# GiulioRomualdi/paper_romualdi_2022_icra_centroidal-mpc-walking

Hardware: AMD Instinct MI355X
Metric: centroidal-MPC solves/sec (batch, horizon=20) (higher is better)
Workload: dtype f32

## Files before the change

### include/cmpc.h

```cpp
#ifndef CMPC_H
#define CMPC_H

#include <stddef.h>

#ifdef __cplusplus
extern "C" {
#endif

typedef struct cmpc_handle_s* cmpc_handle;

typedef enum {
    CMPC_OK = 0,
    CMPC_ERR_ARG = -1,
    CMPC_ERR_HIP = -2,
    CMPC_ERR_NOT_CONVERGED = -3
} cmpc_status;

typedef struct {
    int horizon;
    double sampling_time;
    double friction_coefficient;
    double gravity;
    double com_weight[3];
    double angular_momentum_weight;
// ... 22 lines not shown
void cmpc_default_config(cmpc_config* cfg);
int cmpc_dims(int horizon, int* n_x, int* n_p, int* n_g, int* nnz_jac, int* nnz_hess);

double cmpc_default_tolerance(int horizon);
int cmpc_create(const cmpc_config* cfg, int batch, int device, cmpc_handle* out);
int cmpc_destroy(cmpc_handle h);
const char* cmpc_last_error(cmpc_handle h);
int cmpc_batch(cmpc_handle h);
void* cmpc_stream(cmpc_handle h);

int cmpc_solve_device(cmpc_handle h, const float* dP, const float* dX0, float* dX, float* dInfo,
                      void* stream);
int cmpc_solve_device_warm(cmpc_handle h, const float* dP, const float* dX0, float* dX, float* dInfo,
                           void* stream);
int cmpc_set_warm_policy(cmpc_handle h, int warm_budget, int restart_in_kernel);
int cmpc_solve(cmpc_handle h, const float* P, const float* X0, float* X, float* info);
float cmpc_last_solve_ms(cmpc_handle h);
int cmpc_set_timing(cmpc_handle h, int enabled);
int cmpc_test_poison_lds(cmpc_handle h);

typedef struct {
    double friction_coefficient;
    double com_weight[3];
    double angular_momentum_weight;
    double contact_position_weight;
    double force_rate_of_change_weight[3];
    double contact_force_symmetry_weight;
    double corners[2][4][3];
} cmpc_model;
#define CMPC_MODEL_DOUBLES 34
// ... 137 lines not shown
```

### paper_romualdi_2022_icra_centroidal-mpc-walking_amd/_capi.py

```python
from __future__ import annotations

import ctypes as C
import os

_HERE = os.path.dirname(os.path.abspath(__file__))
LIB_PATH = os.path.join(_HERE, os.environ.get("CMPC_LIB", "libcmpc_hip.so"))

INFO = 8
CERT = 8
SENS = 8


class CmpcConfig(C.Structure):
    _fields_ = [
        ("horizon", C.c_int),
        ("sampling_time", C.c_double),
        ("friction_coefficient", C.c_double),
        ("gravity", C.c_double),
        ("com_weight", C.c_double * 3),
        ("angular_momentum_weight", C.c_double),
        ("contact_position_weight", C.c_double),
        ("force_rate_of_change_weight", C.c_double * 3),
        ("contact_force_symmetry_weight", C.c_double),
        ("corners", C.c_double * 24),
# ... 49 lines not shown
    "cmpc_batch", "cmpc_stream", "cmpc_solve_device", "cmpc_solve", "cmpc_last_solve_ms", "cmpc_set_timing",
    "cmpc_eval_nlp_device", "cmpc_nlp_sparsity", "cmpc_set_state", "cmpc_set_reference",
    "cmpc_set_contacts", "cmpc_set_initial_guess", "cmpc_advance", "cmpc_get_solution",
    "cmpc_get_output", "cmpc_set_reference_from_planner", "cmpc_plant_step_device", "cmpc_test_poison_lds",
    "cmpc_compact_output_device", "cmpc_contacts_merge", "cmpc_contacts_merge_device", "cmpc_contacts_sample",
    "cmpc_contacts_sample_device", "cmpc_set_contact_lists", "cmpc_contacts_adjust", "cmpc_contacts_adjust_device",
    "cmpc_write_state_device", "cmpc_shift_solution_device", "cmpc_eval_nlp_grad_device", "cmpc_solve_device_warm", "cmpc_set_warm_policy",
    "cmpc_get_parameters", "cmpc_get_parameters_device", "cmpc_allgather_compact_device",
    "cmpc_rollout_tick_device", "cmpc_write_reference_from_planner_device", "cmpc_default_tolerance",
    "cmpc_contacts_force_sample_time", "cmpc_contacts_force_sample_time_device",
    "cmpc_model_from_config", "cmpc_check_models", "cmpc_set_models", "cmpc_set_models_device",
    "cmpc_set_multiplier_output", "cmpc_get_multipliers_device", "cmpc_get_multipliers", "cmpc_kkt_certificate_device",
    "cmpc_value_gradient_device", "cmpc_solution_jvp_device", "cmpc_solution_vjp_device",
    "cmpc_sensitivity_workspace_bytes", "cmpc_solution_jvp_model_device", "cmpc_solution_vjp_model_device", "cmpc_model_value_gradient_device",
    "cmpc_plant_step_jvp_device", "cmpc_plant_step_vjp_device", "cmpc_contacts_position_vjp_device", "cmpc_rollout_tick_vjp_device",
]

_lib = None


def lib():
    global _lib
    if _lib is None:
        if not os.path.exists(LIB_PATH):
            raise RuntimeError(
                f"{LIB_PATH} not found: build it with `python -c 'import __graft_entry__ as g; g.build()'` "
                "(hipcc --offload-arch=gfx950). This package has no CPU fallback.")
        try:
            import torch
        except ImportError:
# ... 62 lines not shown
            L.cmpc_solution_jvp_model_device.argtypes = [vp, fp, fp, fp, fp, vp, C.c_int, fp, fp, vp]
            L.cmpc_solution_vjp_model_device.argtypes = [vp, fp, fp, fp, fp, fp, vp, fp, vp]
            L.cmpc_model_value_gradient_device.argtypes = [vp, fp, fp, fp, vp, vp]
        L.cmpc_plant_step_jvp_device.argtypes = [vp, fp, fp, fp, d, i, vp, fp, fp, vp, vp, vp]
        L.cmpc_plant_step_vjp_device.argtypes = [vp, fp, fp, fp, d, i, vp, vp, fp, fp, vp, vp]
        L.cmpc_contacts_position_vjp_device.argtypes = [vp, i, d, i, i] + [vp] * 15
        L.cmpc_rollout_tick_vjp_device.argtypes = [vp, i, d, C.POINTER(CmpcTickTape)] + [vp] * 11
        if hasattr(L, "cmpc_get_parameters"):
            L.cmpc_get_parameters.argtypes = [vp, fp]
            L.cmpc_get_parameters_device.argtypes = [vp, C.POINTER(vp)]
            L.cmpc_allgather_compact_device.argtypes = [vp, vp, C.c_int, fp, fp, vp]
        if hasattr(L, "cmpc_rollout_tick_device"):
            L.cmpc_rollout_tick_device.argtypes = [vp, i, d, i, C.POINTER(CmpcTickIO), vp]
        if hasattr(L, "cmpc_write_reference_from_planner_device"):
            L.cmpc_write_reference_from_planner_device.argtypes = [vp, fp, fp, i, d, d, d, d, fp, vp]
        if hasattr(L, "cmpc_set_models"):
            L.cmpc_model_from_config.argtypes = [C.POINTER(CmpcConfig), C.POINTER(CmpcModel)]
            L.cmpc_model_from_config.restype = None
            L.cmpc_check_models.argtypes = [vp, i]
            L.cmpc_set_models.argtypes = [vp, vp]
            L.cmpc_set_models_device.argtypes = [vp, vp, vp, vp]
        _lib = L
    return _lib
```

### paper_romualdi_2022_icra_centroidal-mpc-walking_amd/csrc/cmpc_api.hip

```cpp
#include "../../include/cmpc.h"
#include "cmpc_contacts.h"
#include "cmpc_device.h"

#include <algorithm>
#include <cmath>
#include <cstdio>
#include <cstdlib>
#include <cstring>
#include <dlfcn.h>
#include <string>
#include <vector>

extern "C" size_t cmpc_solver_lds_bytes(int N, int factors_global);
extern "C" int cmpc_launch_solver(const CmpcParams* prm, size_t lds_bytes, hipStream_t stream);
extern "C" int cmpc_prepare_solver(int N, int factors_global, size_t lds_bytes);
extern "C" int cmpc_launch_nlp_eval(const CmpcParams* prm, const float* dX, const float* dP, const float* dLamG,
                                    float lam_f, float* dF, float* dG, float* dGradF, float* dJac, float* dHess,
                                    hipStream_t stream);
extern "C" int cmpc_launch_nlp_grad(const CmpcParams* prm, const float* dX, const float* dP, const float* dLamG, float lam_f, float* dGradX,
                                    float* dGradP, hipStream_t stream);
extern "C" int cmpc_launch_multipliers(const CmpcParams* prm, const float* dX, const float* dP, float* dLamG, hipStream_t stream);
extern "C" int cmpc_launch_kkt_certificate(const CmpcParams* prm, const float* dX, const float* dP, const float* dLamG, float* dCert, hipStream_t stream);
extern "C" int cmpc_launch_value_gradient(const CmpcParams* prm, const float* dX, const float* dP, const float* dLamG, float* dGradP, hipStream_t stream);
extern "C" int cmpc_launch_sensitivity(const CmpcConsts* kc, int kc_per_problem, int N, int b0, int nb, const float* dX, const float* dP, const float* dLamG,
                                       const float* dDir, const float* dGradX, int kdir, float* dOut, float* dSens, double* dWs, const double* dDirModel,
                                       double* dGradModel, hipStream_t stream);
extern "C" int cmpc_launch_model_value_gradient(const CmpcParams* prm, const float* dX, const float* dP, const float* dLamG, double* dGradModel,
                                                hipStream_t stream);
extern "C" int cmpc_launch_warm_shift(const CmpcParams* prm, const float* dXprev, float* dX0, hipStream_t stream);
extern "C" int cmpc_launch_contacts_merge(int B, int M, double now, const double* plan_t, const float* plan_pose, const int* plan_n,
// ... 37 lines not shown
    CmpcLayout L;
    int B = 0, device = 0;
    hipStream_t stream = nullptr;
    hipEvent_t ev0 = nullptr, ev1 = nullptr;
    bool timed = false;
    bool timing = true;
    float* dP = nullptr;
    float* dX0 = nullptr;
    float* dX = nullptr;
    float* dInfo = nullptr;
    CmpcConsts* dConsts = nullptr;
    double hExpK[CMPC_NMAX + 1];
    double* dExpK = nullptr;
    CmpcConsts* dModels = nullptr;
    bool models_set = false;
    float* dScratch = nullptr;
    float* dBox = nullptr;
    float* dDuals = nullptr;
    bool mult_out = false;
    float* dLamG = nullptr;
    double* dSensWs = nullptr;
    hipEvent_t sens_ev = nullptr;
    double* dSnapT = nullptr;
    int* dSnapOk = nullptr;
    char* dTickWs = nullptr;
    hipEvent_t tick_ev = nullptr;
    size_t snap_cap = 0;
    int warm_duals = 0;
    float hBox[12] = {0};
    bool box_set = false;
// ... 147 lines not shown
    HIPCHK_CREATE(hipMalloc(&h->dConsts, sizeof(CmpcConsts)));
    for (int k = 0; k <= cfg->horizon; ++k) h->hExpK[k] = std::exp(-(double)k);
    HIPCHK_CREATE(hipMalloc(&h->dExpK, sizeof(double) * (cfg->horizon + 1)));
    HIPCHK_CREATE(hipMemcpy(h->dExpK, h->hExpK, sizeof(double) * (cfg->horizon + 1), hipMemcpyHostToDevice));
    HIPCHK_CREATE(hipMalloc(&h->dBox, sizeof(float) * 12));
    if (h->warm_duals) {
        const size_t nd = (size_t)batch * (CMPC_NS * (cfg->horizon + 1) + 2 * CMPC_NI * cfg->horizon);
        HIPCHK_CREATE(hipMalloc(&h->dDuals, sizeof(float) * nd));
        HIPCHK_CREATE(hipMemset(h->dDuals, 0, sizeof(float) * nd));
    }
    {
        CmpcConsts q;
        fill_consts(h, q);
        HIPCHK_CREATE(hipMemcpy(h->dConsts, &q, sizeof(q), hipMemcpyHostToDevice));
    }
    HIPCHK_CREATE(hipDeviceSynchronize());
#undef HIPCHK_CREATE
    *out = h;
    return CMPC_OK;
}

int cmpc_destroy(cmpc_handle h)
{
    if (!h) return CMPC_OK;
    hipSetDevice(h->device);
    if (h->stream) hipStreamSynchronize(h->stream);
    if (h->hXpin) hipHostFree(h->hXpin);
    if (h->hInfoPin) hipHostFree(h->hInfoPin);
    hipFree(h->dP); hipFree(h->dX0); hipFree(h->dX); hipFree(h->dInfo); hipFree(h->dConsts); hipFree(h->dScratch); hipFree(h->dBox); hipFree(h->dDuals); hipFree(h->dLamG); hipFree(h->dSensWs);
    if (h->sens_ev) hipEventDestroy(h->sens_ev);
    hipFree(h->dSnapT); hipFree(h->dSnapOk); hipFree(h->dTickWs); if (h->tick_ev) hipEventDestroy(h->tick_ev); hipFree(h->dExpK); hipFree(h->dModels);
    if (h->ev0) hipEventDestroy(h->ev0);
    if (h->ev1) hipEventDestroy(h->ev1);
    if (h->stream) hipStreamDestroy(h->stream);
    delete h;
    return CMPC_OK;
}

static void fill_consts(cmpc_handle h, CmpcConsts& q)
{
    const cmpc_config& c = h->cfg;
    std::memset(&q, 0, sizeof(q));
    q.N = c.horizon; q.max_iter = c.max_iterations;
    q.exact_hessian = c.exact_hessian; q.final_extrap = c.final_extrapolation;
    q.tail_stages = c.tail_stages; q.tail_iters = c.tail_iterations; q.tail_trigger = (float)c.tail_trigger;
    q.dt = (float)c.sampling_time; q.grav = (float)c.gravity;
// ... 9 lines not shown
    q.sigma_min = 0.03f;
#ifdef CMPC_PROFILE
    if (const char* e = std::getenv("CMPC_SIGMA_MIN")) q.sigma_min = (float)std::atof(e);
    if (const char* e = std::getenv("CMPC_HWID_PROBE")) q.hwid_probe = std::atoi(e);
#endif
}

static const float* model_corners(cmpc_handle h) { return h->models_set ? h->dModels->corners : h->dConsts->corners; }
static int corners_stride(cmpc_handle h) { return h->models_set ? (int)(sizeof(CmpcConsts) / sizeof(float)) : 0; }

static void fill_params(cmpc_handle h, CmpcParams& p)
{
    std::memset(&p, 0, sizeof(p));
    p.kc = h->models_set ? h->dModels : h->dConsts; p.N = h->cfg.horizon; p.B = h->B;
    p.kc_per_problem = h->models_set ? 1 : 0;
    p.scratch = h->dScratch; p.scratch_stride = h->scratch_stride;
    p.mu_init = h->cfg.mu_init > 0 ? (float)h->cfg.mu_init : 0.1f;
    p.mu_adapt = h->cfg.mu_init > 0 ? 0.f : h->mu_adapt;
    p.t_floor = 1e-2f;
    p.warm_budget = h->warm_budget; p.warm_no_restart = h->warm_no_restart;
    p.duals = (h->mult_out || h->warm_duals) ? h->dDuals : nullptr; p.warm_duals = h->warm_duals;
}

static int solve_device_impl(cmpc_handle h, const float* dP, const float* dX0, float* dX, float* dInfo, void* stream, bool warm)
{
    if (!h || !dP || !dX0 || !dX) return fail(h, CMPC_ERR_ARG, "cmpc_solve_device: null argument");
    HIPCHK(h, hipSetDevice(h->device));
    hipStream_t st = stream ? (hipStream_t)stream : h->stream;
    CmpcParams p;
    fill_params(h, p);
    p.P = dP; p.X0 = dX0; p.X = dX; p.info = dInfo ? dInfo : h->dInfo;
    if (warm || h->force_warm) {
        p.mu_init = (float)h->mu_warm; p.mu_adapt = 0.f; p.t_floor = (float)h->floor_warm; p.warm = 1;
    }
    if (h->timing) HIPCHK(h, hipEventRecord(h->ev0, st));
    int rc = cmpc_launch_solver(&p, h->lds, st);
    if (rc != 0) return fail(h, CMPC_ERR_HIP, std::string("solver launch: ") + hipGetErrorString((hipError_t)rc));
    if (h->timing) HIPCHK(h, hipEventRecord(h->ev1, st));
    h->timed = h->timing;
    return CMPC_OK;
}

int cmpc_solve_device(cmpc_handle h, const float* dP, const float* dX0, float* dX, float* dInfo, void* stream)
{
    return solve_device_impl(h, dP, dX0, dX, dInfo, stream, false);
}

int cmpc_set_warm_policy(cmpc_handle h, int warm_budget, int restart_in_kernel)
{
    if (!h || warm_budget < 0) return fail(h, CMPC_ERR_ARG, "cmpc_set_warm_policy: bad argument");
    h->warm_budget = warm_budget;
    h->warm_no_restart = restart_in_kernel ? 0 : 1;
    return CMPC_OK;
}

int cmpc_solve_device_warm(cmpc_handle h, const float* dP, const float* dX0, float* dX, float* dInfo, void* stream)
{
    return solve_device_impl(h, dP, dX0, dX, dInfo, stream, true);
}

// ... 1002 lines not shown
```

### paper_romualdi_2022_icra_centroidal-mpc-walking_amd/csrc/cmpc_device.h

```cpp
#pragma once
#include <hip/hip_runtime.h>

#include "../../include/cmpc.h"

#define CMPC_NS 15
#define CMPC_NF 24
#define CMPC_NQ 6
#define CMPC_NU 30
#define CMPC_NXA 39
#define CMPC_NI 44
#define CMPC_REC_N 1088
#define CMPC_NMAX 40
#define CMPC_TZ_LDS_NMAX 20
#define CMPC_INFO_N 8

struct CmpcLayout {
    int N;
    int p_R[2], p_up[2], p_lo[2], p_gam[2], p_nom[2], p_cur[2];
    int p_com0, p_dcom0, p_h0, p_comref, p_href, p_fext, p_text, np;
    int o_com, o_dcom, o_h, o_pos[2], o_vel[2], o_f[2][4], nx, ng;
};

__host__ __device__ inline void cmpc_layout_init(CmpcLayout& L, int N)
{
// ... 108 lines not shown
    const float* P;
    const float* X0;
    float* X;
    float* info;
    float mu_init, t_floor;
    float mu_adapt;
    int warm;
    int warm_budget;
    int warm_no_restart;
    float* duals;
    int warm_duals;
    float* scratch;
    long long scratch_stride;
    int lds_words;
    int kc_per_problem;
};
```

### paper_romualdi_2022_icra_centroidal-mpc-walking_amd/csrc/cmpc_solver.hip

```cpp
#include "cmpc_device.h"

#include <cstdlib>
#include <type_traits>
#include <map>
#include <mutex>

#define NS CMPC_NS
#define NF CMPC_NF
#define NQ CMPC_NQ
#define NU CMPC_NU
#define NXA CMPC_NXA
#define NI CMPC_NI
#define PLD 39
#define GLD 30
#define RLD 36
#define NPAN 46
#define GEO 36
#define SQ_TILE_WAVES 6
#define SQ_SPIN_MAX (1 << 20)
#define SQ_PUB_FLOATS (10 * NPAN * 4 + 128 * 4)
#define ZLD 36
#define MSET (NU * RLD + NPAN * RLD + NS * 16)
#define NTRI 256
#define ID_STRIP_LEN 68
// ... 63 lines not shown
    float *S, *U, *T, *Z;
    float* LAM;
    float *dS, *dU, *dT, *dZ, *d;
    float *Lf;
    float *geoA;
    float *P0, *Qb, *G, *QuuF, *Pan, *Bval, *Aval, *arow, *ybuf, *fpv, *fpn;
    float *idstrip;
    float *ZT;
    double *QuuD1, *qs1;
    int *Brow, *Arow, *qmask;
    unsigned short* tri;
    double *QuuD, *pv, *pn, *qs, *Pd, *sig, *gco, *redd;
    float* red;
    int* flag;
    int* prog;
};

__device__ inline void wave_lds_sync() { asm volatile("" ::: "memory"); }
typedef __attribute__((address_space(3))) const float* ldsf_t;
typedef __attribute__((address_space(3))) float* ldsw_t;
__device__ inline ldsf_t lds_opaque(const float* p) { ldsf_t q = (ldsf_t)p; asm volatile("" : "+v"(q)); return q; }
__device__ inline ldsw_t lds_opaque_w(float* p) { ldsw_t q = (ldsw_t)p; asm volatile("" : "+v"(q)); return q; }
typedef float v4f __attribute__((ext_vector_type(4)));
typedef float v2f __attribute__((ext_vector_type(2)));
__device__ inline float4 lds_ld4(ldsf_t p)
{
    const v4f v = *reinterpret_cast<__attribute__((address_space(3))) const v4f*>(p);
    return make_float4(v[0], v[1], v[2], v[3]);
}

// ... 73 lines not shown
    if (!FG) { c.Lf = fp; fp += (size_t)REC_N * N; } else c.Lf = fg_base;
    c.sp = fp; fp += (c.L.np() + 3) & ~3;
    c.S = fp; fp += NS * (N + 1); c.U = fp; fp += NU * N;
    if (!FG || N <= CMPC_TZ_LDS_NMAX) { c.T = fp; fp += NI * N; c.Z = fp; fp += NI * N; }
    else { c.T = fg_base + (size_t)REC_N * N; c.Z = c.T + NI * N; }
    c.d = fp; fp += NS * N;
    c.LAM = fp; fp += NS * (N + 1);
    c.geoA = fp; fp += GEO * N;
    c.Bval = fp; fp += 3 * NU; c.Aval = fp; fp += 3 * NS + 3;
    c.arow = fp; fp += 96 + 12; fp += DSET_F;
    c.fpv = fp; fp += 40; c.fpn = fp; fp += 40; c.red = fp; fp += 24;
    c.Brow = reinterpret_cast<int*>(fp); fp += 3 * NU;
    c.Arow = reinterpret_cast<int*>(fp); fp += 3 * NS + 3; fp += DSET_I;
    c.flag = reinterpret_cast<int*>(fp); fp += 4;
    c.prog = c.flag;
    if (!FG) { c.prog = reinterpret_cast<int*>(fp); fp += 128; }
    c.qmask = reinterpret_cast<int*>(fp); fp += CMPC_NMAX;
    c.tri = reinterpret_cast<unsigned short*>(fp); fp += NTRI / 2;
}

__device__ inline void use_desc_set(Ctx& c, int s)
{
    c.Bval += s * DSET_F; c.Aval += s * DSET_F; c.arow += s * DSET_F;
    c.Brow += s * DSET_I; c.Arow += s * DSET_I;
    c.sig += s * 2 * NI; c.gco += s * 2 * NI;
}

__device__ inline int ub_row(int m) { const int I = m >> 2; return REC_UB + 16 * (8 * I - I * (I - 1) / 2) + (m & 3) * 4 * (8 - I); }
__device__ inline int wt_idx(int j, int a) { return REC_WT + 32 * j + 4 * ((a >> 2) ^ (j & 7)) + (a & 3); }
__device__ inline float half_sum(float v)
{
// ... 197 lines not shown
__device__ inline float wave_max(float v)
{
    v = fmaxf(v, dpp_f<0xB1>(v));
    v = fmaxf(v, dpp_f<0x4E>(v));
    v = fmaxf(v, dpp_f<0x141>(v));
    v = fmaxf(v, dpp_f<0x140>(v));
    return fmaxf(fmaxf(readlane_f(v, 0), readlane_f(v, 16)), fmaxf(readlane_f(v, 32), readlane_f(v, 48)));
}
__device__ inline double wave_sum(double v)
{
    v += dpp_d<0xB1>(v);
    v += dpp_d<0x4E>(v);
    v += dpp_d<0x141>(v);
    v += dpp_d<0x140>(v);
    return (readlane_d(v, 0) + readlane_d(v, 16)) + (readlane_d(v, 32) + readlane_d(v, 48));
}
template <int NT, int NV>
__device__ inline void block_maxn(float (&v)[NV], float* red, int tid)
{
#pragma unroll
    for (int q = 0; q < NV; ++q) v[q] = wave_max(v[q]);
    __syncthreads();
    if ((tid & 63) == 0) {
#pragma unroll
        for (int q = 0; q < NV; ++q) red[3 * (tid >> 6) + q] = v[q];
    }
    __syncthreads();
#pragma unroll
    for (int q = 0; q < NV; ++q) {
        float r = red[q];
// ... 843 lines not shown
        char* smk = (char*)lk;
        Ctx c;
        make_ctx<FG>(c, smk, N, fg_base);
        const CmpcConsts& prm = *reinterpret_cast<const CmpcConsts*>(smk);
        const int s = k & 1;
        const int fixedmask = (~c.qmask[k]) & 63;
        SQPROF_DECL;
        stage_factor<FG, true>(c.QuuF + s * MSET, s ? c.QuuD1 : c.QuuD, c.Pan + s * MSET, RecRef<FG>(c.Lf, N, k), c.idstrip, prm.D, c.flag, tid,
                                     fixedmask, c.ZT, c.prog + tid, 16 * ord);
        SQPROF(9);
        __syncthreads();
        SQPROF(3);
    }
    __builtin_amdgcn_s_setprio(0);
}
struct ConsPlan {
    int t_dst, t_w, t_y0, t_y1, t_y2, t_e;
    float t_symk, t_fsel, t_esgn, t_efsel, t_qdc, t_zsel, t_m0, t_m1, t_m2;
    int pa0, pa1, pa2, pa3, pb0, pb1, pb2, pb3, wa, wb;
    float wa3, wb3;
    int d0, d1, d2, d3;
    int ri[14];
    float rf[6];
};
#define SQ_TRASH (32)
__device__ inline void plan_rows(const int* rows, int col, int& r0, int& r1, int& r2) { r0 = rows[3 * col]; r1 = rows[3 * col + 1]; r2 = rows[3 * col + 2]; }
__device__ inline void cons_plan_build(ConsPlan& pl, const Ctx& c, const CmpcConsts& prm, int w7, int ln, const int* rows)
{
    const int wv = w7 < 4 ? w7 - 1 : w7 - 2;
    const int m4 = ln & 15, kq = ln >> 4;
    {
        const int id = (wv >= 0 && w7 != 4) ? 64 * wv + ln : 360;
        const bool val = id < 360;
        const int idc = val ? id : 0;
        const bool isuu = idc < 135, isss = idc >= 285;
        const int p = isuu ? idc / 3 : 0;
        const int bi = 1 + (p >= 1) + (p >= 3) + (p >= 6) + (p >= 10) + (p >= 15) + (p >= 21) + (p >= 28) + (p >= 36);
        const int bj = p - bi * (bi - 1) / 2;
        const int idp = isuu ? 0 : (isss ? idc - 285 : idc - 135);
// ... 46 lines not shown
                if (ii >= NU) {
                    if (jj < NU) { p = NU * RLD + (ii - NU) * RLD + jj; p2 = p; }
                    else { p = NU * RLD + NPAN * RLD + 16 * (ii - NU) + (jj - NU); p2 = NU * RLD + NPAN * RLD + 16 * (jj - NU) + (ii - NU); }
                }
                d[i] = ok ? p : SQ_TRASH + i; e[i] = ok ? p2 : SQ_TRASH + i;
            }
        };
        results(I, J, wv >= 0 && wv < 5);
        pl.d0 = d[0]; pl.d1 = d[1]; pl.d2 = d[2]; pl.d3 = d[3];
        if (wv == 3) results(1, 1, true);
    }
#pragma unroll
    for (int q = 0; q < 14; ++q) pl.ri[q] = 0;
#pragma unroll
    for (int q = 0; q < 6; ++q) pl.rf[q] = 0.f;
    if (wv == 0) {
        const int tc = ln < 60 ? ln : 59;
        const int b = tc / 6, w = tc - 6 * b;
        const int rr = w >= 3 ? 2 : (w >= 1 ? 1 : 0), cc = w - rr * (rr + 1) / 2;
        const int i = 3 * b + rr, j = 3 * b + cc;
        const bool isF = i < NF;
        int r0, r1, r2;
        plan_rows(rows, i, r0, r1, r2);
        const int f0 = isF ? 4 * b : 0;
        pl.ri[0] = 3 * i; pl.ri[1] = 16 * j + r0; pl.ri[2] = 16 * j + r1; pl.ri[3] = 16 * j + r2;
        pl.ri[4] = f0; pl.ri[5] = 3 * f0 + rr; pl.ri[6] = 3 * f0 + cc; pl.ri[7] = isF ? 0 : i - 24;
        pl.ri[8] = 9 * b + 3 * rr + cc;
        pl.ri[9] = i * RLD + j;
        pl.rf[0] = isF ? 1.f : 0.f; pl.rf[1] = rr == cc ? 1.f : 0.f; pl.rf[2] = (isF && i >= 12) ? 1.f : 0.f; pl.rf[3] = prm.D[i % 3];
    } else if (wv == 1) {
// ... 339 lines not shown
                Mn[pl.ri[5]] = r0; Mn[pl.ri[6]] = r1; Mn[pl.ri[7]] = r2; Mn[pl.ri[8]] = r3;
                Mn[pl.ri[9]] = r0; Mn[pl.ri[10]] = r1; Mn[pl.ri[11]] = r2; Mn[pl.ri[12]] = r3;
            }
        }
        CPROF(4);
    }
    if (gaveup && ln == 0) sq_give_up(c);
}
template <int NT, int NC, bool FG>
__device__ __attribute__((noinline)) void sq_consume_loop(lds_t lds, int Nrt, float* fg_base, int k0_in, bool exact_in, float reg, float cmu)
{
    CMPC_PHASE_PROLOGUE;
    const int k0 = __builtin_amdgcn_readfirstlane(k0_in);
    const bool use_exact = __builtin_amdgcn_readfirstlane((int)exact_in) != 0;
    ConsPlan pl;
    cons_plan_build(pl, c, prm, tid >> 6, tid & 63, c.Brow + ((N - 1) & 1) * DSET_I);
    sq_consume_stage(c, prm, pl, tid, N, N, N - 1, -1, 0, false, use_exact, reg, cmu);
    __syncthreads();
    int ord = 0;
#pragma unroll 1
    for (int k = N - 1; k >= k0; --k) {
        ++ord;
        if (k > k0) sq_consume_stage(c, prm, pl, tid, N, k, k - 1, k - 2 >= k0 ? k - 2 : -1, ord, true, use_exact, reg, cmu);
        __syncthreads();
    }
}
template <int NT, int NC, bool FG>
__device__ __attribute__((noinline)) void sq_init(lds_t lds, int Nrt, float* fg_base, int k0_in, bool exact_in, float cmu)
{
    CMPC_PHASE_PROLOGUE;
    const int k0 = __builtin_amdgcn_readfirstlane(k0_in);
// ... 789 lines not shown
    const int k0 = (prm.tail_stages > 0 && m3[1] > prm.tail_trigger * m3[2]) ? kt : N;
    if (k0 < N) step_lengths<NT>(c, tid, 0.999f, ap, ad, 0, k0);
    for (int e = tid; e < NS * (k0 < N ? k0 + 1 : N + 1); e += NT) c.S[e] += ap * c.dS[e];
    for (int e = tid; e < NU * k0; e += NT) c.U[e] += ap * c.dU[e];
    if (duals)
        for (int e = tid; e < NI * k0; e += NT) {
            const float tn = c.T[e] + ap * c.dT[e], zn = dual_extrapolate(c.Z[e], c.dZ[e]);
            if (fabsf(tn) < INFINITY && fabsf(zn) < INFINITY) { c.T[e] = tn; c.Z[e] = zn; }
        }
    __syncthreads();
    if (k0 == N) return false;
    tail_polish<NT, NC, FG>(lds, N, fg_base, k0, duals);
    return true;
}

template <int NT, int NC, bool FG>
__device__ __attribute__((noinline)) int phase_setup(lds_t lds, int Nrt, float* fg_base, const float* gp)
{
    CMPC_PHASE_PROLOGUE;
    float* spw = const_cast<float*>(c.sp);
    for (int e = tid; e < NTRI; e += NT) {
        int i = (int)((sqrtf(8.f * (float)e + 1.f) - 1.f) * 0.5f);
        while ((i + 1) * (i + 2) / 2 <= e) ++i;
        while (i * (i + 1) / 2 > e) --i;
        c.tri[e] = (unsigned short)((i << 8) | (e - i * (i + 1) / 2));
    }
    for (int e = tid; e < ID_STRIPS; e += NT) c.idstrip[e] = (e % ID_STRIP_LEN) == 32 + e / ID_STRIP_LEN ? 1.f : 0.f;
    for (int e = tid; e < c.L.np(); e += NT) spw[e] = gp[e];
    if (tid == 0) c.flag[0] = 0;
    __syncthreads();
    if (tid < N) {
        int m = 0;
#pragma unroll
        for (int q = 0; q < NQ; ++q) m |= qfree_compute(c, tid, q) ? (1 << q) : 0;
        c.qmask[tid] = m;
    }
    if (tid < 2 * N && outside_subset(c, tid / N, tid % N)) c.flag[0] = 1;
    __syncthreads();
    return __builtin_amdgcn_readfirstlane(c.flag[0]);
}

template <int NT, int NC, bool FG>
__device__ __attribute__((noinline)) int phase_init(lds_t lds, int Nrt, float* fg_base, const float* x0, const float* dprev, int flags, float mu_init,
                                                    float t_floor)
// ... 33 lines not shown
        const int k = e / NI, i = e % NI;
        float t = 1.f, z = 0.f;
        if (row_active(c, k, i)) {
            t = -row_val(c, prm, k, i, c.U + NU * k);
            if (i < 32) t = fmaxf(t, t_floor);
            z = mu_init / t;
            if (use_mult && !cold) {
                const int kk = k + 1 < N ? k + 1 : N - 1;
                z = fmaxf(z, dprev[NS * (N + 1) + NI * N + NI * kk + i]);
            }
        }
        c.T[e] = t; c.Z[e] = z;
    }
    __syncthreads();
    int nrow = 0;
    for (int k = 0; k < N; ++k)
        for (int i = 32; i < NI; ++i) nrow += row_active(c, k, i) ? 1 : 0;
    return __builtin_amdgcn_readfirstlane(nrow + 32 * N);
}

template <int NT, int NC, bool FG>
__device__ __attribute__((noinline)) float phase_multipliers(lds_t lds, int Nrt, float* fg_base, int mode_in, float a_in, int nrow_in)
{
    CMPC_PHASE_PROLOGUE;
    const int mode = __builtin_amdgcn_readfirstlane(mode_in), nrow = __builtin_amdgcn_readfirstlane(nrow_in);
    const float a = uniform_f(a_in);
    float out = a;
    if (mode == 0) {
        for (int e = tid; e < NI * N; e += NT) c.Z[e] *= a;
    } else if (mode == 1) {
        double l2 = 0.0;
        for (int e = tid; e < NI * N; e += NT)
            if (row_active(c, e / NI, e % NI)) {
// ... 216 lines not shown
#ifdef CMPC_PROFILE
    if (prm.hwid_probe) {
        __syncthreads();
        if ((threadIdx.x & 63) == 0) x[threadIdx.x >> 6] = (float)(__builtin_amdgcn_s_getreg((31 << 11) | 4) & 0xffff);
    }
#endif
}

template <int NT, int NC, bool FG>
__global__ __launch_bounds__(NT, FG ? 3 : 1) void cmpc_solve_kernel(CmpcParams kp)
{
    extern __shared__ __attribute__((aligned(16))) char smem[];
    const int b = blockIdx.x;
    const int tid = threadIdx.x;
    const int N = NC > 0 ? NC : kp.N;
    {
        int* z = reinterpret_cast<int*>(smem);
        for (int e = tid; e < kp.lds_words; e += NT) z[e] = 0;
    }
    __syncthreads();
    {
        const int* src = reinterpret_cast<const int*>(kp.kc_per_problem ? kp.kc + b : kp.kc);
        int* dst = reinterpret_cast<int*>(smem);
        for (int e = tid; e < (int)(sizeof(CmpcConsts) / 4); e += NT) dst[e] = src[e];
    }
    const CmpcConsts& prm = *reinterpret_cast<const CmpcConsts*>(smem);
    const long long t_start = __builtin_amdgcn_s_memtime();
    unsigned ldsv = (unsigned)(unsigned long long)(lds_t)smem;
    asm volatile("" : "+s"(ldsv));
    const lds_t lds = (lds_t)(unsigned long long)ldsv;
    float* const fg_base = FG ? kp.scratch + (size_t)b * kp.scratch_stride : nullptr;
    const CmpcIdx L{N};
    __syncthreads();
    const bool outside = (phase_setup<NT, NC, FG>(lds, N, fg_base, kp.P + (size_t)b * L.np()) != 0) | (prm.model_bad != 0);
    int status = 1, sg = 0, it_total = 0;
    float err = 0.f, ep = 0.f, mu_cur = 0.f, step_out = 0.f, step_prev = 0.f;
    float* const dq = kp.duals ? kp.duals + (size_t)b * (NS * (N + 1) + 2 * NI * N) : nullptr;
    if (outside) {
        phase_init<NT, NC, FG>(lds, N, fg_base, kp.X0 + (size_t)b * L.nx(), dq, 0, kp.mu_init, kp.t_floor);
        status = 3;
    }
    for (int pass = 0; pass < 2 && !outside; ++pass) {
        const float mu_init = pass ? 0.1f : kp.mu_init, t_floor = pass ? 1e-2f : kp.t_floor, mu_adapt = pass ? 3.5f : kp.mu_adapt;
        step_out = step_prev = 0.f;
        const bool use_duals = kp.warm && kp.warm_duals && kp.duals;
        const int nrow = phase_init<NT, NC, FG>(lds, N, fg_base, kp.X0 + (size_t)b * L.nx(), dq,
                                                (pass > 0 ? 1 : 0) | (use_duals ? 2 : 0) | (use_duals && kp.warm_duals > 1 ? 4 : 0), mu_init, t_floor);
        int it = 0;
        status = 1;
// ... 102 lines not shown
            }
        }
        it_total += it;
        if (status == 0 || !kp.warm || pass > 0 || kp.warm_no_restart) break;
        sg += 10000;
        __syncthreads();
    }
    phase_export<NT, NC, FG>(lds, N, fg_base, kp.X + (size_t)b * L.nx(), dq, status);
    if (kp.info && tid == 0) {
        float* inf = kp.info + (size_t)b * CMPC_INFO_N;
        inf[0] = (float)it_total; inf[1] = err; inf[2] = mu_cur; inf[3] = (float)sg; inf[4] = ep; inf[5] = (float)status;
        inf[6] = (float)(__builtin_amdgcn_s_memtime() - t_start); inf[7] = step_out;
    }
}

}

extern "C" size_t cmpc_solver_lds_bytes(int N, int factors_global)
{
    CmpcLayout L;
    cmpc_layout_init(L, N);
    const size_t dbl = 90 + 40 + 40 + 16 + 40 + 4 * NI + 8 + (factors_global ? 0 : 90 + 16);
    const size_t work = factors_global ? ((NXA * PLD + 3) & ~3) + NS * 16 + ((NXA * GLD + 3) & ~3) : (size_t)MSET + NS * 16 + SQ_PUB_FLOATS + 128;
    const size_t flt = (size_t)NU * RLD + (size_t)NPAN * RLD + 96 + ID_STRIPS + ((L.np + 3) & ~3)
                       + ((size_t)NS * (N + 1) + (size_t)NU * N + ((factors_global && N > CMPC_TZ_LDS_NMAX) ? 0 : 2 * (size_t)NI * N)) + (size_t)NS * N + (size_t)NS * (N + 1)
                       + (size_t)GEO * N + work + 2 * DSET_F + 40 + 40 + 24
                       + 2 * DSET_I + 4 + CMPC_NMAX + NTRI / 2 + (factors_global ? 0 : (size_t)REC_N * N);
    return ((sizeof(CmpcConsts) + 15) & ~(size_t)15) + dbl * 8 + flt * 4;
}

#ifdef CMPC_PROFILE
extern "C" int cmpc_profile_read(long long* out, int reset)
{
    hipError_t e = hipMemcpyFromSymbol(out, HIP_SYMBOL(g_prof), sizeof(long long) * 128);
    if (reset) { long long z[128] = {0}; (void)hipMemcpyToSymbol(HIP_SYMBOL(g_prof), z, sizeof(z)); }
    return (int)e;
}
extern "C" int cmpc_trace_read(float* out) { return (int)hipMemcpyFromSymbol(out, HIP_SYMBOL(g_trace), sizeof(float) * 64 * 8); }
#endif

typedef void (*cmpc_kernel_t)(CmpcParams);
static cmpc_kernel_t solver_variant(int N, bool factors_global, int& nthreads)
// ... 43 lines not shown
```

### paper_romualdi_2022_icra_centroidal-mpc-walking_amd/solver.py

```python
from __future__ import annotations

import ctypes as C
from typing import Dict, List, Optional, Sequence

import numpy as np

from . import _capi
from .config import GRAVITY, CentroidalMPCConfig, from_ini, model_array
from .contacts import PlannedContact, pack_lists, sample_schedule, sample_schedule_batch
from .layout import Layout


def _c_config(cfg: CentroidalMPCConfig, tolerance=None, mu_min=None, max_iterations=None,
              exact_hessian=True, final_extrapolation=True, step_tolerance=None, mu_init=None,
              tail_stages=3, tail_iterations=2, tail_trigger=2e-5, factors=None) -> _capi.CmpcConfig:
    c = _capi.CmpcConfig()
    c.horizon = cfg.N
    c.sampling_time = cfg.sampling_time
    c.friction_coefficient = cfg.static_friction_coefficient
    c.gravity = GRAVITY
    c.com_weight[:] = cfg.com_weight
    c.angular_momentum_weight = cfg.angular_momentum_weight
    c.contact_position_weight = cfg.contact_position_weight
    c.force_rate_of_change_weight[:] = cfg.force_rate_of_change_weight
# ... 112 lines not shown

    def set_models_device(self, models, ok=None):
        import torch
        assert models.is_cuda and models.dtype == torch.float64 and models.is_contiguous() and tuple(models.shape) == (self.batch, _capi.MODEL_DOUBLES)
        if ok is None:
            ok = torch.empty((self.batch,), dtype=torch.int32, device=models.device)
        assert ok.dtype == torch.int32 and ok.is_contiguous() and ok.numel() == self.batch
        self._launch(models.device, lambda st: self._lib.cmpc_set_models_device(self._h, models.data_ptr(), ok.data_ptr(), st))
        return ok

    def set_warm_policy(self, warm_budget: int = 0, restart_in_kernel: bool = True):
        rc = self._lib.cmpc_set_warm_policy(self._h, int(warm_budget), 1 if restart_in_kernel else 0)
        if rc != 0:
            raise RuntimeError(f"cmpc_set_warm_policy failed ({rc}): {self.last_error}")

    def last_solve_ms(self) -> float:
        return float(self._lib.cmpc_last_solve_ms(self._h))

    def set_timing(self, enabled: bool = True):
        if hasattr(self._lib, "cmpc_set_timing"):
            self._lib.cmpc_set_timing(self._h, 1 if enabled else 0)

    def compact_output_device(self, dX, dInfo, out=None):
        import torch
        W = 3 * (self.cfg.N + 1) + 38
        if out is None:
            out = torch.empty((self.batch, W), dtype=torch.float32, device=dX.device)
        assert out.is_contiguous() and tuple(out.shape) == (self.batch, W)
        st, cur = self._stream_pair(dX.device)
        rc = self._lib.cmpc_compact_output_device(self._h, dX.data_ptr(), dInfo.data_ptr(), out.data_ptr(), st)
# ... 547 lines not shown
```

Measured before the change: 352,800.

## Precompute constraint plans and LDS lookup tables once per handle

Adds a one-time kernel at handle creation that builds the triangle-index table, identity strips and per-lane constraint plans into a global blob. Each solve then copies these with vectorized loads instead of recomputing them per block, and the row count becomes a wave-parallel popcount instead of a serial double loop. LDS zeroing now uses int4 stores and skips the consts region. The tables are only valid when a single shared model is in use, so they are turned off when per-problem models are set, and they cost an extra global buffer plus LDS words.

```diff
diff --git a/include/cmpc.h b/include/cmpc.h
--- a/include/cmpc.h
+++ b/include/cmpc.h
@@ -60,6 +60,7 @@
 int cmpc_solve_device_warm(cmpc_handle h, const float* dP, const float* dX0, float* dX, float* dInfo,
                            void* stream);
 int cmpc_set_warm_policy(cmpc_handle h, int warm_budget, int restart_in_kernel);
+int cmpc_set_plan_tables(cmpc_handle h, int enabled);
 int cmpc_solve(cmpc_handle h, const float* P, const float* X0, float* X, float* info);
 float cmpc_last_solve_ms(cmpc_handle h);
 int cmpc_set_timing(cmpc_handle h, int enabled);
diff --git a/paper_romualdi_2022_icra_centroidal-mpc-walking_amd/_capi.py b/paper_romualdi_2022_icra_centroidal-mpc-walking_amd/_capi.py
--- a/paper_romualdi_2022_icra_centroidal-mpc-walking_amd/_capi.py
+++ b/paper_romualdi_2022_icra_centroidal-mpc-walking_amd/_capi.py
@@ -87,6 +87,7 @@
     "cmpc_value_gradient_device", "cmpc_solution_jvp_device", "cmpc_solution_vjp_device",
     "cmpc_sensitivity_workspace_bytes", "cmpc_solution_jvp_model_device", "cmpc_solution_vjp_model_device", "cmpc_model_value_gradient_device",
     "cmpc_plant_step_jvp_device", "cmpc_plant_step_vjp_device", "cmpc_contacts_position_vjp_device", "cmpc_rollout_tick_vjp_device",
+    "cmpc_set_plan_tables",
 ]
 
 _lib = None
@@ -179,6 +180,8 @@
             L.cmpc_rollout_tick_device.argtypes = [vp, i, d, i, C.POINTER(CmpcTickIO), vp]
         if hasattr(L, "cmpc_write_reference_from_planner_device"):
             L.cmpc_write_reference_from_planner_device.argtypes = [vp, fp, fp, i, d, d, d, d, fp, vp]
+        if hasattr(L, "cmpc_set_plan_tables"):
+            L.cmpc_set_plan_tables.argtypes = [vp, C.c_int]
         if hasattr(L, "cmpc_set_models"):
             L.cmpc_model_from_config.argtypes = [C.POINTER(CmpcConfig), C.POINTER(CmpcModel)]
             L.cmpc_model_from_config.restype = None
diff --git a/paper_romualdi_2022_icra_centroidal-mpc-walking_amd/csrc/cmpc_api.hip b/paper_romualdi_2022_icra_centroidal-mpc-walking_amd/csrc/cmpc_api.hip
--- a/paper_romualdi_2022_icra_centroidal-mpc-walking_amd/csrc/cmpc_api.hip
+++ b/paper_romualdi_2022_icra_centroidal-mpc-walking_amd/csrc/cmpc_api.hip
@@ -14,6 +14,8 @@
 extern "C" size_t cmpc_solver_lds_bytes(int N, int factors_global);
 extern "C" int cmpc_launch_solver(const CmpcParams* prm, size_t lds_bytes, hipStream_t stream);
 extern "C" int cmpc_prepare_solver(int N, int factors_global, size_t lds_bytes);
+extern "C" size_t cmpc_plan_tables_words(void);
+extern "C" int cmpc_build_plan_tables(const CmpcConsts* kc, int N, int resident, size_t lds_bytes, unsigned* out, hipStream_t stream);
 extern "C" int cmpc_launch_nlp_eval(const CmpcParams* prm, const float* dX, const float* dP, const float* dLamG,
                                     float lam_f, float* dF, float* dG, float* dGradF, float* dJac, float* dHess,
                                     hipStream_t stream);
@@ -81,6 +83,8 @@
     double* dExpK = nullptr;
     CmpcConsts* dModels = nullptr;
     bool models_set = false;
+    unsigned* dTables = nullptr;
+    bool plan_tables = true;
     float* dScratch = nullptr;
     float* dBox = nullptr;
     float* dDuals = nullptr;
@@ -258,6 +262,9 @@
         fill_consts(h, q);
         HIPCHK_CREATE(hipMemcpy(h->dConsts, &q, sizeof(q), hipMemcpyHostToDevice));
     }
+    HIPCHK_CREATE(hipMalloc(&h->dTables, sizeof(unsigned) * cmpc_plan_tables_words()));
+    HIPCHK_CREATE(hipMemset(h->dTables, 0, sizeof(unsigned) * cmpc_plan_tables_words()));
+    HIPCHK_CREATE((hipError_t)cmpc_build_plan_tables(h->dConsts, cfg->horizon, fg ? 0 : 1, h->lds, h->dTables, nullptr));
     HIPCHK_CREATE(hipDeviceSynchronize());
 #undef HIPCHK_CREATE
     *out = h;
@@ -273,7 +280,7 @@
     if (h->hInfoPin) hipHostFree(h->hInfoPin);
     hipFree(h->dP); hipFree(h->dX0); hipFree(h->dX); hipFree(h->dInfo); hipFree(h->dConsts); hipFree(h->dScratch); hipFree(h->dBox); hipFree(h->dDuals); hipFree(h->dLamG); hipFree(h->dSensWs);
     if (h->sens_ev) hipEventDestroy(h->sens_ev);
-    hipFree(h->dSnapT); hipFree(h->dSnapOk); hipFree(h->dTickWs); if (h->tick_ev) hipEventDestroy(h->tick_ev); hipFree(h->dExpK); hipFree(h->dModels);
+    hipFree(h->dSnapT); hipFree(h->dSnapOk); hipFree(h->dTickWs); if (h->tick_ev) hipEventDestroy(h->tick_ev); hipFree(h->dExpK); hipFree(h->dModels); hipFree(h->dTables);
     if (h->ev0) hipEventDestroy(h->ev0);
     if (h->ev1) hipEventDestroy(h->ev1);
     if (h->stream) hipStreamDestroy(h->stream);
@@ -313,6 +320,7 @@
     std::memset(&p, 0, sizeof(p));
     p.kc = h->models_set ? h->dModels : h->dConsts; p.N = h->cfg.horizon; p.B = h->B;
     p.kc_per_problem = h->models_set ? 1 : 0;
+    p.tables = (h->plan_tables && !h->models_set) ? h->dTables : nullptr;
     p.scratch = h->dScratch; p.scratch_stride = h->scratch_stride;
     p.mu_init = h->cfg.mu_init > 0 ? (float)h->cfg.mu_init : 0.1f;
     p.mu_adapt = h->cfg.mu_init > 0 ? 0.f : h->mu_adapt;
@@ -343,6 +351,13 @@
 int cmpc_solve_device(cmpc_handle h, const float* dP, const float* dX0, float* dX, float* dInfo, void* stream)
 {
     return solve_device_impl(h, dP, dX0, dX, dInfo, stream, false);
+}
+
+int cmpc_set_plan_tables(cmpc_handle h, int enabled)
+{
+    if (!h) return fail(h, CMPC_ERR_ARG, "cmpc_set_plan_tables: null handle");
+    h->plan_tables = enabled != 0;
+    return CMPC_OK;
 }
 
 int cmpc_set_warm_policy(cmpc_handle h, int warm_budget, int restart_in_kernel)
diff --git a/paper_romualdi_2022_icra_centroidal-mpc-walking_amd/csrc/cmpc_device.h b/paper_romualdi_2022_icra_centroidal-mpc-walking_amd/csrc/cmpc_device.h
--- a/paper_romualdi_2022_icra_centroidal-mpc-walking_amd/csrc/cmpc_device.h
+++ b/paper_romualdi_2022_icra_centroidal-mpc-walking_amd/csrc/cmpc_device.h
@@ -146,4 +146,5 @@
     long long scratch_stride;
     int lds_words;
     int kc_per_problem;
+    const unsigned* tables;
 };
diff --git a/paper_romualdi_2022_icra_centroidal-mpc-walking_amd/csrc/cmpc_solver.hip b/paper_romualdi_2022_icra_centroidal-mpc-walking_amd/csrc/cmpc_solver.hip
--- a/paper_romualdi_2022_icra_centroidal-mpc-walking_amd/csrc/cmpc_solver.hip
+++ b/paper_romualdi_2022_icra_centroidal-mpc-walking_amd/csrc/cmpc_solver.hip
@@ -101,6 +101,7 @@
     float* red;
     int* flag;
     int* prog;
+    int* ptab;
 };
 
 __device__ inline void wave_lds_sync() { asm volatile("" ::: "memory"); }
@@ -204,7 +205,8 @@
     c.Arow = reinterpret_cast<int*>(fp); fp += 3 * NS + 3; fp += DSET_I;
     c.flag = reinterpret_cast<int*>(fp); fp += 4;
     c.prog = c.flag;
-    if (!FG) { c.prog = reinterpret_cast<int*>(fp); fp += 128; }
+    c.ptab = c.flag;
+    if (!FG) { c.prog = reinterpret_cast<int*>(fp); fp += 128; c.ptab = reinterpret_cast<int*>(fp); fp += 4; }
     c.qmask = reinterpret_cast<int*>(fp); fp += CMPC_NMAX;
     c.tri = reinterpret_cast<unsigned short*>(fp); fp += NTRI / 2;
 }
@@ -432,6 +434,16 @@
     v += dpp_d<0x141>(v);
     v += dpp_d<0x140>(v);
     return (readlane_d(v, 0) + readlane_d(v, 16)) + (readlane_d(v, 32) + readlane_d(v, 48));
+}
+template <int CTRL>
+__device__ inline int dpp_i(int v) { return __builtin_amdgcn_update_dpp(0, v, CTRL, 0xF, 0xF, true); }
+__device__ inline int wave_sum_i(int v)
+{
+    v += dpp_i<0xB1>(v);
+    v += dpp_i<0x4E>(v);
+    v += dpp_i<0x141>(v);
+    v += dpp_i<0x140>(v);
+    return (__builtin_amdgcn_readlane(v, 0) + __builtin_amdgcn_readlane(v, 16)) + (__builtin_amdgcn_readlane(v, 32) + __builtin_amdgcn_readlane(v, 48));
 }
 template <int NT, int NV>
 __device__ inline void block_maxn(float (&v)[NV], float* red, int tid)
@@ -1305,6 +1317,12 @@
     }
     __builtin_amdgcn_s_setprio(0);
 }
+#define TAB_TRI 0
+#define TAB_ID (TAB_TRI + NTRI / 2)
+#define TAB_PLAN (TAB_ID + ID_STRIPS)
+#define PLAN_LANES (7 * 64)
+#define PLAN_VEC 13
+#define TAB_WORDS (TAB_PLAN + PLAN_VEC * 4 * PLAN_LANES)
 struct ConsPlan {
     int t_dst, t_w, t_y0, t_y1, t_y2, t_e;
     float t_symk, t_fsel, t_esgn, t_efsel, t_qdc, t_zsel, t_m0, t_m1, t_m2;
@@ -1313,7 +1331,10 @@
     int d0, d1, d2, d3;
     int ri[14];
     float rf[6];
+    int pad;
 };
+static_assert(sizeof(ConsPlan) == PLAN_VEC * 16, "a ConsPlan is PLAN_VEC 16-byte vectors");
+static_assert(TAB_ID % 4 == 0 && TAB_PLAN % 4 == 0, "the parts of the blob start on 16-byte boundaries");
 #define SQ_TRASH (32)
 __device__ inline void plan_rows(const int* rows, int col, int& r0, int& r1, int& r2) { r0 = rows[3 * col]; r1 = rows[3 * col + 1]; r2 = rows[3 * col + 2]; }
 __device__ inline void cons_plan_build(ConsPlan& pl, const Ctx& c, const CmpcConsts& prm, int w7, int ln, const int* rows)
@@ -1390,6 +1411,7 @@
     for (int q = 0; q < 14; ++q) pl.ri[q] = 0;
 #pragma unroll
     for (int q = 0; q < 6; ++q) pl.rf[q] = 0.f;
+    pl.pad = 0;
     if (wv == 0) {
         const int tc = ln < 60 ? ln : 59;
         const int b = tc / 6, w = tc - 6 * b;
@@ -1759,7 +1781,16 @@
     const int k0 = __builtin_amdgcn_readfirstlane(k0_in);
     const bool use_exact = __builtin_amdgcn_readfirstlane((int)exact_in) != 0;
     ConsPlan pl;
-    cons_plan_build(pl, c, prm, tid >> 6, tid & 63, c.Brow + ((N - 1) & 1) * DSET_I);
+    const unsigned long long tab_a = ((unsigned long long)(unsigned)__builtin_amdgcn_readfirstlane(c.ptab[1]) << 32) | (unsigned)__builtin_amdgcn_readfirstlane(c.ptab[0]);
+    if (tab_a) {
+        typedef __attribute__((address_space(1))) const v4u* gtab_t;
+        const gtab_t src = (gtab_t)(tab_a + 4ull * TAB_PLAN) + (tid - 64);
+        v4u w[PLAN_VEC];
+#pragma unroll
+        for (int q = 0; q < PLAN_VEC; ++q) w[q] = src[q * PLAN_LANES];
+        __builtin_memcpy(&pl, w, sizeof(pl));
+    } else
+        cons_plan_build(pl, c, prm, tid >> 6, tid & 63, c.Brow + ((N - 1) & 1) * DSET_I);
     sq_consume_stage(c, prm, pl, tid, N, N, N - 1, -1, 0, false, use_exact, reg, cmu);
     __syncthreads();
     int ord = 0;
@@ -2579,20 +2610,52 @@
     return true;
 }
 
+__device__ inline unsigned short tri_entry(int e)
+{
+    int i = (int)((sqrtf(8.f * (float)e + 1.f) - 1.f) * 0.5f);
+    while ((i + 1) * (i + 2) / 2 <= e) ++i;
+    while (i * (i + 1) / 2 > e) --i;
+    return (unsigned short)((i << 8) | (e - i * (i + 1) / 2));
+}
+__device__ inline float idstrip_entry(int e) { return (e % ID_STRIP_LEN) == 32 + e / ID_STRIP_LEN ? 1.f : 0.f; }
+template <int NT>
+__device__ inline void copy_words(void* dst_, const void* src_, int n, int tid)
+{
+    int* dst = reinterpret_cast<int*>(dst_);
+    const int* src = reinterpret_cast<const int*>(src_);
+    int n4 = 0;
+    if ((((unsigned long long)src | (unsigned long long)dst) & 15) == 0) {
+        n4 = n >> 2;
+        for (int e = tid; e < n4; e += NT) reinterpret_cast<int4*>(dst)[e] = reinterpret_cast<const int4*>(src)[e];
+    }
+    for (int e = 4 * n4 + tid; e < n; e += NT) dst[e] = src[e];
+}
+template <typename T>
+__device__ inline T* uniform_ptr(T* p)
+{
+    const unsigned long long a = (unsigned long long)p;
+    const unsigned lo = __builtin_amdgcn_readfirstlane((unsigned)a), hi = __builtin_amdgcn_readfirstlane((unsigned)(a >> 32));
+    return (T*)(((unsigned long long)hi << 32) | lo);
+}
+
 template <int NT, int NC, bool FG>
-__device__ __attribute__((noinline)) int phase_setup(lds_t lds, int Nrt, float* fg_base, const float* gp)
+__device__ __attribute__((noinline)) int phase_setup(lds_t lds, int Nrt, float* fg_base, const float* gp, const unsigned* tab_in)
 {
     CMPC_PHASE_PROLOGUE;
     float* spw = const_cast<float*>(c.sp);
-    for (int e = tid; e < NTRI; e += NT) {
-        int i = (int)((sqrtf(8.f * (float)e + 1.f) - 1.f) * 0.5f);
-        while ((i + 1) * (i + 2) / 2 <= e) ++i;
-        while (i * (i + 1) / 2 > e) --i;
-        c.tri[e] = (unsigned short)((i << 8) | (e - i * (i + 1) / 2));
-    }
-    for (int e = tid; e < ID_STRIPS; e += NT) c.idstrip[e] = (e % ID_STRIP_LEN) == 32 + e / ID_STRIP_LEN ? 1.f : 0.f;
-    for (int e = tid; e < c.L.np(); e += NT) spw[e] = gp[e];
-    if (tid == 0) c.flag[0] = 0;
+    const unsigned* tab = uniform_ptr(tab_in);
+    if (tab) {
+        copy_words<NT>(c.tri, tab + TAB_TRI, NTRI / 2, tid);
+        copy_words<NT>(c.idstrip, tab + TAB_ID, ID_STRIPS, tid);
+    } else {
+        for (int e = tid; e < NTRI; e += NT) c.tri[e] = tri_entry(e);
+        for (int e = tid; e < ID_STRIPS; e += NT) c.idstrip[e] = idstrip_entry(e);
+    }
+    copy_words<NT>(spw, gp, c.L.np(), tid);
+    if (tid == 0) {
+        c.flag[0] = 0;
+        if (!FG) { c.ptab[0] = (int)(unsigned)(unsigned long long)tab; c.ptab[1] = (int)(unsigned)((unsigned long long)tab >> 32); }
+    }
     __syncthreads();
     if (tid < N) {
         int m = 0;
@@ -2656,9 +2719,8 @@
     }
     __syncthreads();
     int nrow = 0;
-    for (int k = 0; k < N; ++k)
-        for (int i = 32; i < NI; ++i) nrow += row_active(c, k, i) ? 1 : 0;
-    return __builtin_amdgcn_readfirstlane(nrow + 32 * N);
+    for (int k = tid & 63; k < N; k += 64) nrow += 2 * __builtin_popcount(c.qmask[k] & 63);
+    return wave_sum_i(nrow) + 32 * N;
 }
 
 template <int NT, int NC, bool FG>
@@ -2905,16 +2967,16 @@
     const int b = blockIdx.x;
     const int tid = threadIdx.x;
     const int N = NC > 0 ? NC : kp.N;
+    constexpr int KWORDS = ((sizeof(CmpcConsts) + 15) & ~15) / 4;
     {
+        int4* z4 = reinterpret_cast<int4*>(smem);
+        const int n4 = kp.lds_words >> 2;
+        for (int e = KWORDS / 4 + tid; e < n4; e += NT) z4[e] = make_int4(0, 0, 0, 0);
         int* z = reinterpret_cast<int*>(smem);
-        for (int e = tid; e < kp.lds_words; e += NT) z[e] = 0;
-    }
-    __syncthreads();
-    {
-        const int* src = reinterpret_cast<const int*>(kp.kc_per_problem ? kp.kc + b : kp.kc);
-        int* dst = reinterpret_cast<int*>(smem);
-        for (int e = tid; e < (int)(sizeof(CmpcConsts) / 4); e += NT) dst[e] = src[e];
-    }
+        for (int e = 4 * n4 + tid; e < kp.lds_words; e += NT) z[e] = 0;
+        if (tid < KWORDS - (int)(sizeof(CmpcConsts) / 4)) z[sizeof(CmpcConsts) / 4 + tid] = 0;
+    }
+    copy_words<NT>(smem, kp.kc_per_problem ? kp.kc + b : kp.kc, (int)(sizeof(CmpcConsts) / 4), tid);
     const CmpcConsts& prm = *reinterpret_cast<const CmpcConsts*>(smem);
     const long long t_start = __builtin_amdgcn_s_memtime();
     unsigned ldsv = (unsigned)(unsigned long long)(lds_t)smem;
@@ -2923,7 +2985,7 @@
     float* const fg_base = FG ? kp.scratch + (size_t)b * kp.scratch_stride : nullptr;
     const CmpcIdx L{N};
     __syncthreads();
-    const bool outside = (phase_setup<NT, NC, FG>(lds, N, fg_base, kp.P + (size_t)b * L.np()) != 0) | (prm.model_bad != 0);
+    const bool outside = (phase_setup<NT, NC, FG>(lds, N, fg_base, kp.P + (size_t)b * L.np(), kp.tables) != 0) | (prm.model_bad != 0);
     int status = 1, sg = 0, it_total = 0;
     float err = 0.f, ep = 0.f, mu_cur = 0.f, step_out = 0.f, step_prev = 0.f;
     float* const dq = kp.duals ? kp.duals + (size_t)b * (NS * (N + 1) + 2 * NI * N) : nullptr;
@@ -3056,6 +3118,56 @@
     }
 }
 
+__global__ __launch_bounds__(512, 1) void cmpc_plan_tables_kernel(const CmpcConsts* kc, int N, int with_plans, int lds_words, unsigned* out)
+{
+    extern __shared__ __attribute__((aligned(16))) char smem[];
+    constexpr int NT = 512;
+    const int tid = threadIdx.x;
+    unsigned short* tri = reinterpret_cast<unsigned short*>(out + TAB_TRI);
+    for (int e = tid; e < NTRI; e += NT) tri[e] = tri_entry(e);
+    float* ids = reinterpret_cast<float*>(out + TAB_ID);
+    for (int e = tid; e < ID_STRIPS; e += NT) ids[e] = idstrip_entry(e);
+    if (!with_plans) return;
+    {
+        int* z = reinterpret_cast<int*>(smem);
+        for (int e = tid; e < lds_words; e += NT) z[e] = 0;
+    }
+    __syncthreads();
+    copy_words<NT>(smem, kc, (int)(sizeof(CmpcConsts) / 4), tid);
+    __syncthreads();
+    Ctx c;
+    make_ctx<false>(c, smem, N, nullptr);
+    const CmpcConsts& prm = *reinterpret_cast<const CmpcConsts*>(smem);
+    if (tid >= 384) {
+        Ctx cd = c;
+        use_desc_set(cd, (N - 1) & 1);
+        stage_desc_body(cd, prm, desc_pack_t(tid & 127), N - 1, false, 0.f);
+    }
+    __syncthreads();
+    if (tid >= 64) {
+        ConsPlan pl;
+        cons_plan_build(pl, c, prm, tid >> 6, tid & 63, c.Brow + ((N - 1) & 1) * DSET_I);
+        v4u w[PLAN_VEC];
+        __builtin_memcpy(w, &pl, sizeof(pl));
+        v4u* dst = reinterpret_cast<v4u*>(out + TAB_PLAN) + (tid - 64);
+#pragma unroll
+        for (int q = 0; q < PLAN_VEC; ++q) dst[q * PLAN_LANES] = w[q];
+    }
+}
+
+}
+
+extern "C" size_t cmpc_plan_tables_words(void) { return TAB_WORDS; }
+extern "C" int cmpc_build_plan_tables(const CmpcConsts* kc, int N, int resident, size_t lds_bytes, unsigned* out, hipStream_t stream)
+{
+    const size_t lds = resident ? lds_bytes : 0;
+    (void)hipGetLastError();
+    if (lds > 48 * 1024) {
+        const hipError_t e = hipFuncSetAttribute(reinterpret_cast<const void*>(cmpc_plan_tables_kernel), hipFuncAttributeMaxDynamicSharedMemorySize, (int)lds);
+        if (e != hipSuccess) return (int)e;
+    }
+    hipLaunchKernelGGL(cmpc_plan_tables_kernel, dim3(1), dim3(512), lds, stream, kc, N, resident ? 1 : 0, (int)(lds / 4), out);
+    return (int)hipGetLastError();
 }
 
 extern "C" size_t cmpc_solver_lds_bytes(int N, int factors_global)
@@ -3067,7 +3179,7 @@
     const size_t flt = (size_t)NU * RLD + (size_t)NPAN * RLD + 96 + ID_STRIPS + ((L.np + 3) & ~3)
                        + ((size_t)NS * (N + 1) + (size_t)NU * N + ((factors_global && N > CMPC_TZ_LDS_NMAX) ? 0 : 2 * (size_t)NI * N)) + (size_t)NS * N + (size_t)NS * (N + 1)
                        + (size_t)GEO * N + work + 2 * DSET_F + 40 + 40 + 24
-                       + 2 * DSET_I + 4 + CMPC_NMAX + NTRI / 2 + (factors_global ? 0 : (size_t)REC_N * N);
+                       + 2 * DSET_I + 4 + (factors_global ? 0 : 4) + CMPC_NMAX + NTRI / 2 + (factors_global ? 0 : (size_t)REC_N * N);
     return ((sizeof(CmpcConsts) + 15) & ~(size_t)15) + dbl * 8 + flt * 4;
 }
 
diff --git a/paper_romualdi_2022_icra_centroidal-mpc-walking_amd/solver.py b/paper_romualdi_2022_icra_centroidal-mpc-walking_amd/solver.py
--- a/paper_romualdi_2022_icra_centroidal-mpc-walking_amd/solver.py
+++ b/paper_romualdi_2022_icra_centroidal-mpc-walking_amd/solver.py
@@ -150,6 +150,11 @@
         if rc != 0:
             raise RuntimeError(f"cmpc_set_warm_policy failed ({rc}): {self.last_error}")
 
+    def set_plan_tables(self, enabled: bool = True):
+        rc = self._lib.cmpc_set_plan_tables(self._h, 1 if enabled else 0)
+        if rc != 0:
+            raise RuntimeError(f"cmpc_set_plan_tables failed ({rc}): {self.last_error}")
+
     def last_solve_ms(self) -> float:
         return float(self._lib.cmpc_last_solve_ms(self._h))
 
```

Result: no change. 352,000 (-0.2%).
